# Arthur151/ROMP

Measured on NVIDIA H100. Metric: frames/sec 512x512 ROMP-HRNet32 (whole hot path), higher is better.
Workload: dtype bf16

## Files before the change

### romp_b200/csrc/conv_block_tc.cu

```cuda
#include "conv_tc.cuh"
#include "tc_device.cuh"

namespace b200romp {

namespace {

constexpr int kBlkThreads = 384;
constexpr int kRowB = 128;
constexpr int kHaloH = 20;
constexpr int kTapBytes = 64 * kRowB;
constexpr int kHalfTapBytes = 64 * 64;

template <bool FOLD>
struct BlkCfg {
  static constexpr int kWBytes = FOLD ? 3 * (kTapBytes + 2 * kHalfTapBytes) : 9 * kTapBytes;
  static constexpr int kTW = FOLD ? 16 : 8;
  static constexpr int kHaloW = kTW + 4;
  static constexpr int kN1 = FOLD ? 192 : 128;
  static constexpr int kN2 = 8 * kTW;
  static constexpr int kG2 = kN2 / 8;
  static constexpr int kMidRows = 2 * kN1;
  static constexpr int kStagePayload = kHaloH * kHaloW * kRowB;
  static constexpr int kStageBytes = ((kMidRows + 2 * kHaloW + 2) * kRowB + 1023) / 1024 * 1024;
  static constexpr int kMidBytes = kMidRows * kRowB;
  static constexpr int kSmemBytes = 2 * kWBytes + kStageBytes + kMidBytes + 1024  + 1024 ;
  static_assert(17 * kHaloW + kTW + 1 < kMidRows, "conv1 blocks do not cover the mid pixels conv2 reads");
  static_assert(kHaloH * kHaloW - 2 * kHaloW - 2 > 17 * kHaloW + kTW + 1, "an unwritten stage row feeds a mid row conv2 reads");
  static_assert(kSmemBytes <= 227 * 1024, "fused block does not fit shared memory");
  static_assert(kWBytes % kTapBytes == 0, "weights are copied in tap-sized pieces");
};

__host__ __device__ constexpr int w_tap_off(bool fold, int tap) {
  return !fold ? tap * kTapBytes
               : (tap / 3) * (kTapBytes + 2 * kHalfTapBytes) + (tap % 3 == 0 ? 0 : tap % 3 == 1 ? kHalfTapBytes : kHalfTapBytes + kTapBytes);
}

template <bool FOLD>
__device__ __forceinline__ constexpr bool blk_skip(int tap, int k) {
  return FOLD && ((tap % 3 == 0 && k < 2) || (tap % 3 == 2 && k >= 2));
}

template <bool FOLD>
__device__ __forceinline__ uint64_t w_desc(uint32_t w_base, int tap, int k) {
  const uint32_t t = w_base + (uint32_t)w_tap_off(FOLD, tap);
  if (FOLD && tap % 3 != 1) return make_smem_desc(t + (k & 1) * 32, 8 * 64, kSw64);
  return make_smem_desc(t + k * 32, 8 * kRowB, kSw128);
}

__device__ __forceinline__ void consumers_bar_sync() { asm volatile("bar.sync 1, 256;" ::: "memory"); }

__device__ __forceinline__ void ldmatrix_x4_trans(uint32_t (&r)[4], uint32_t addr) {
  asm volatile("ldmatrix.sync.aligned.m8n8.x4.trans.shared.b16 {%0, %1, %2, %3}, [%4];"
               : "=r"(r[0]), "=r"(r[1]), "=r"(r[2]), "=r"(r[3])
               : "r"(addr));
}
__device__ __forceinline__ void stmatrix_x4_trans(uint32_t addr, const uint32_t (&r)[4]) {
  asm volatile("stmatrix.sync.aligned.m8n8.x4.trans.shared.b16 [%0], {%1, %2, %3, %4};" ::"r"(addr), "r"(r[0]), "r"(r[1]), "r"(r[2]),
               "r"(r[3])
               : "memory");
}
__device__ __forceinline__ void st_shared_zero16(uint32_t addr) {
  asm volatile("st.shared.v4.b32 [%0], {%1, %1, %1, %1};" ::"r"(addr), "r"(0) : "memory");
}
template <int N>
__device__ __forceinline__ void wgmma_bf16(float (&d)[N / 2], uint64_t a, uint64_t b, uint32_t scale_d) {
  if constexpr (N == 192) wgmma_n192_bf16(d, a, b, scale_d);
  else if constexpr (N == 128) wgmma_n128_bf16(d, a, b, scale_d);
  else wgmma_n64(d, a, b, scale_d, false);
}
template <typename T>
__device__ __forceinline__ T opaque(T v) {
  uint64_t u = (uint64_t)v;
  asm volatile("mov.b64 %0, %0;" : "+l"(u));
  return (T)u;
}
__device__ __forceinline__ uint32_t pack_bf16x2(float a, float b) {
  const __nv_bfloat162 v = __floats2bfloat162_rn(a, b);
  return *reinterpret_cast<const uint32_t*>(&v);
}

struct BlkThread {
  int g, w, l;
};
template <bool FOLD>
__device__ __forceinline__ int c2_oy0(int g) { return FOLD ? 0 : 8 * g; }
template <bool FOLD>
__device__ __forceinline__ int c2_ox0(int g) { return FOLD ? 8 * g : 0; }
struct BlkTile {
  int n, y0, x0;
  __device__ BlkTile(int tile, int tiles_x, int per_frame, int tw) {
    n = tile / per_frame;
    const int rem = tile % per_frame;
    y0 = (rem / tiles_x) * 16;
    x0 = (rem % tiles_x) * tw;
  }
};

template <bool FOLD>
__device__ __forceinline__ void conv1_issue(float (&acc)[BlkCfg<FOLD>::kN1 / 2], uint32_t a_base, uint32_t w1_base, int row0) {
  constexpr int kHaloW = BlkCfg<FOLD>::kHaloW, kN1 = BlkCfg<FOLD>::kN1;
#pragma unroll
  for (int j = 0; j < kN1 / 2; ++j) acc[j] = 0.f;
  uint32_t scale_d = 0;
  wgmma_fence();
#pragma unroll
  for (int tap = 0; tap < 9; ++tap) {
    const uint32_t b_tap = a_base + (uint32_t)((row0 + (tap / 3) * kHaloW + tap % 3) * kRowB);
#pragma unroll
    for (int k = 0; k < 4; ++k) {
      if (blk_skip<FOLD>(tap, k)) continue;
      wgmma_bf16<kN1>(acc, w_desc<FOLD>(w1_base, tap, k), make_smem_desc(b_tap + k * 32, 8 * kRowB, kSw128), scale_d);
      scale_d = 1;
    }
  }
  wgmma_commit();
}

template <bool FOLD>
__device__ __forceinline__ void load_residual(uint32_t (&rv)[BlkCfg<FOLD>::kG2][2], uint32_t a_base, const BlkThread& th) {
  constexpr int kHaloW = BlkCfg<FOLD>::kHaloW;
  const int q = th.l >> 3;
#pragma unroll
  for (int j0 = 0; j0 < BlkCfg<FOLD>::kG2; j0 += 2) {
    const int hr = (c2_oy0<FOLD>(th.g) + j0 + (q >> 1) + 2) * kHaloW + c2_ox0<FOLD>(th.g) + (th.l & 7) + 2;
    uint32_t r[4];
    ldmatrix_x4_trans(r, a_base + hr * kRowB + (((2 * th.w + (q & 1)) ^ (hr & 7)) << 4));
    rv[j0][0] = r[0]; rv[j0][1] = r[1]; rv[j0 + 1][0] = r[2]; rv[j0 + 1][1] = r[3];
  }
}

template <bool FOLD>
__device__ __forceinline__ void mid_epilogue(const float (&acc)[BlkCfg<FOLD>::kN1 / 2], uint32_t mid_base, const float* b1p, const ConvParams& p,
                                             const BlkTile& tl, const BlkThread& th, int row0) {
  constexpr int kHaloW = BlkCfg<FOLD>::kHaloW, kTW = BlkCfg<FOLD>::kTW, kN1 = BlkCfg<FOLD>::kN1;
  const float bias[2] = {__ldg(b1p + 16 * th.w + (th.l >> 2)), __ldg(b1p + 16 * th.w + (th.l >> 2) + 8)};
  const int q = th.l >> 3;
#pragma unroll
  for (int j0 = 0; j0 < kN1 / 8; j0 += 2) {
    uint32_t r[4];
#pragma unroll
    for (int i = 0; i < 4; ++i) {
      const int j = j0 + (i >> 1), e = i & 1;
      r[i] = pack_bf16x2(fmaxf(acc[4 * j + 2 * e] + bias[e], 0.f), fmaxf(acc[4 * j + 2 * e + 1] + bias[e], 0.f));
    }
    const int m = row0 + 8 * (j0 + (q >> 1)) + (th.l & 7);
    stmatrix_x4_trans(mid_base + m * kRowB + (((2 * th.w + (q & 1)) ^ (m & 7)) << 4), r);
  }
  if (tl.y0 > 0 && tl.x0 > 0 && tl.y0 + 16 < p.Hout && tl.x0 + kTW < p.Wout) return;
  __syncwarp();
  constexpr int kRingRow = kTW + 2, kRing = 2 * kRingRow + 2 * 18;
#pragma unroll 1
  for (int i = th.l; i < 2 * kRing; i += 32) {
    const int k = i >> 1;
    const int my = k < 2 * kRingRow ? (k < kRingRow ? 0 : 17) : (k - 2 * kRingRow) % 18;
    const int mx = k < 2 * kRingRow ? k % kRingRow : (k - 2 * kRingRow < 18 ? 0 : kTW + 1);
    const int m = my * kHaloW + mx;
    if (m >= row0 && m < row0 + kN1 && ((unsigned)(tl.y0 - 1 + my) >= (unsigned)p.Hout || (unsigned)(tl.x0 - 1 + mx) >= (unsigned)p.Wout))
      st_shared_zero16(mid_base + m * kRowB + (((2 * th.w + (i & 1)) ^ (m & 7)) << 4));
  }
}

template <bool FOLD>
__device__ __forceinline__ void conv2_issue(float (&acc2)[BlkCfg<FOLD>::kN2 / 2], uint32_t mid_base, uint32_t w2_base, int g) {
  constexpr int kHaloW = BlkCfg<FOLD>::kHaloW, kN2 = BlkCfg<FOLD>::kN2;
#pragma unroll
  for (int j = 0; j < kN2 / 2; ++j) acc2[j] = 0.f;
  uint32_t scale_d = 0;
  wgmma_fence();
#pragma unroll
  for (int tap = 0; tap < 9; ++tap) {
    const uint32_t b_tap = mid_base + (uint32_t)(((c2_oy0<FOLD>(g) + tap / 3) * kHaloW + c2_ox0<FOLD>(g) + tap % 3) * kRowB);
#pragma unroll
    for (int k = 0; k < 4; ++k) {
      if (blk_skip<FOLD>(tap, k)) continue;
      wgmma_bf16<kN2>(acc2, w_desc<FOLD>(w2_base, tap, k), make_smem_desc(b_tap + k * 32, kHaloW * kRowB, kSw128), scale_d);
      scale_d = 1;
    }
  }
  wgmma_commit();
}

template <bool FOLD>
__device__ __forceinline__ void out_epilogue(const float (&acc2)[BlkCfg<FOLD>::kN2 / 2], const uint32_t (&rv)[BlkCfg<FOLD>::kG2][2],
                                             const float* b2p, const ConvParams& p, const BlkTile& tl, const BlkThread& th) {
  __nv_bfloat16* out = reinterpret_cast<__nv_bfloat16*>(p.out);
  const int c = 16 * th.w + (th.l >> 2);
  const float bias[2] = {__ldg(b2p + c), __ldg(b2p + c + 8)};
  const int odd = (th.l >> 2) & 1;
  const int x = tl.x0 + c2_ox0<FOLD>(th.g) + 2 * (th.l & 3) + odd;
#pragma unroll
  for (int j = 0; j < BlkCfg<FOLD>::kG2; ++j) {
    uint16_t h[2][2];
#pragma unroll
    for (int e = 0; e < 2; ++e) {
      const float2 r = res_pair(rv[j][e]);
      const float a = (acc2[4 * j + 2 * e] + bias[e]) + r.x, b = (acc2[4 * j + 2 * e + 1] + bias[e]) + r.y;
      h[e][0] = __bfloat16_as_ushort(__float2bfloat16_rn(fmaxf(a, 0.f)));
      h[e][1] = __bfloat16_as_ushort(__float2bfloat16_rn(fmaxf(b, 0.f)));
    }
    const uint32_t send = odd ? (uint32_t)h[0][0] | ((uint32_t)h[1][0] << 16) : (uint32_t)h[0][1] | ((uint32_t)h[1][1] << 16);
    const uint32_t recv = __shfl_xor_sync(0xffffffffu, send, 4);
    const size_t pix = ((size_t)tl.n * p.Hout + tl.y0 + c2_oy0<FOLD>(th.g) + j) * p.Wout + x;
    uint32_t* o = reinterpret_cast<uint32_t*>(out + pix * p.out_C + p.out_c_off + (c & ~1));
#pragma unroll
    for (int e = 0; e < 2; ++e) {
      const uint32_t theirs = (recv >> (16 * e)) & 0xFFFFu;
      o[4 * e] = odd ? (theirs | ((uint32_t)h[e][1] << 16)) : ((uint32_t)h[e][0] | (theirs << 16));
    }
  }
}

}

template <bool FOLD>
__global__ void __launch_bounds__(kBlkThreads, 1)
conv_block_tc_kernel(const __grid_constant__ CUtensorMap tmap, const ConvParams p, const uint8_t* __restrict__ w1pack,
                     const uint8_t* __restrict__ w2pack, const float* __restrict__ bias1, int tiles_x, int tiles_y, int num_tiles) {
  using Cfg = BlkCfg<FOLD>;
  constexpr int kWBytes = Cfg::kWBytes, kStageBytes = Cfg::kStageBytes;
  extern __shared__ uint8_t smem_raw[];
  uint8_t* smem = reinterpret_cast<uint8_t*>((reinterpret_cast<uintptr_t>(smem_raw) + 1023) & ~(uintptr_t)1023);
  uint8_t* sW1 = smem;
  uint8_t* sW2 = smem + kWBytes;
  uint8_t* sA = smem + 2 * kWBytes;
  uint8_t* sMid = sA + kStageBytes;
  uint64_t* full = reinterpret_cast<uint64_t*>(sMid + Cfg::kMidBytes);
  uint64_t* empty = full + 1;
  uint64_t* w_full = full + 2;

  const int warp = threadIdx.x >> 5;
  if (threadIdx.x == 0) {
    mbar_init(full, 1);
    mbar_init(empty, 256);
    mbar_init(w_full, 1);
    fence_barrier_init();
  }
  __syncthreads();
  pdl_trigger();
  const int per_frame = tiles_x * tiles_y;

  if (warp == 0) {
    if (elect_one()) {
      mbar_arrive_expect_tx(w_full, 2 * kWBytes);
      for (int off = 0; off < kWBytes; off += kTapBytes) {
        bulk_copy_g2s(sW1 + off, w1pack + off, kTapBytes, w_full);
        bulk_copy_g2s(sW2 + off, w2pack + off, kTapBytes, w_full);
      }
      pdl_wait();
      const uint64_t pol = l2_policy_stream();
      uint32_t phase = 0;
      for (int tile = blockIdx.x; tile < num_tiles; tile += gridDim.x, phase ^= 1) {
        const BlkTile tl(tile, tiles_x, per_frame, Cfg::kTW);
        mbar_wait(empty, phase ^ 1);
        mbar_arrive_expect_tx(full, Cfg::kStagePayload);
        tma_load_4d(sA, &tmap, full, 0, tl.x0 - 2, tl.y0 - 2, tl.n, pol);
      }
    }
  } else if (warp >= 4) {
    const int t = threadIdx.x & 127;
    const BlkThread th{(warp >> 2) - 1, t >> 5, t & 31};
    pdl_wait();
    mbar_wait(w_full, 0);
    float acc[Cfg::kN1 / 2], acc2[Cfg::kN2 / 2];
    uint32_t rv[Cfg::kG2][2];
    const int row0 = th.g * Cfg::kN1;
    uint32_t phase = 0;
    for (int tile = blockIdx.x; tile < num_tiles; tile += gridDim.x, phase ^= 1) {
      const uint32_t w1_base = opaque(smem_u32(sW1)), w2_base = opaque(smem_u32(sW2)), a_base = opaque(smem_u32(sA)),
                     mid_base = opaque(smem_u32(sMid));
      const float* b1p = opaque(bias1);
      const float* b2p = opaque(p.bias);
      const BlkTile tl(tile, tiles_x, per_frame, Cfg::kTW);
      mbar_wait(full, phase);
      conv1_issue<FOLD>(acc, a_base, w1_base, row0);
      load_residual<FOLD>(rv, a_base, th);
      wgmma_wait<0>();
      mbar_arrive(empty);
      consumers_bar_sync();
      mid_epilogue<FOLD>(acc, mid_base, b1p, p, tl, th, row0);
      fence_proxy_async();
      consumers_bar_sync();
      conv2_issue<FOLD>(acc2, mid_base, w2_base, th.g);
      wgmma_wait<0>();
      out_epilogue<FOLD>(acc2, rv, b2p, p, tl, th);
    }
  }
}

bool tc_block_supported(const ConvParams& p, bool fold) {
  if (p.in_dtype != B200ROMP_BF16 || p.out_dtype != B200ROMP_BF16 || p.res_dtype != B200ROMP_BF16) return false;
  if (p.cin != 64 || p.cout != 64 || p.up != 1 || p.out_nchw || p.pow_channel >= 0 || p.input_norm || !p.relu) return false;
  if (p.Hin != p.Hout || p.Win != p.Wout || p.Hout % 16 != 0 || p.Wout % (fold ? BlkCfg<true>::kTW : BlkCfg<false>::kTW) != 0) return false;
  if (p.in_C % 8 != 0 || p.in_c_off % 8 != 0 || p.out_C % 8 != 0 || p.out_c_off % 8 != 0) return false;
  if (p.res != p.in || p.res_C != p.in_C || p.res_c_off != p.in_c_off || p.res_broadcast) return false;
  return (reinterpret_cast<uintptr_t>(p.in) & 15) == 0;
}

static int block_pack_weights(const float* w_oihw, bool fold, void** d_out, std::vector<void*>* allocs) {
  if (!fold) return tc_pack_weights(w_oihw, 64, 64, 9, 64, d_out, allocs, kRowB, 2);
  const std::vector<uint8_t> full = tc_pack_image(w_oihw, 64, 64, 9, 64, kRowB, 2);
  const std::vector<uint8_t> half = tc_pack_image(w_oihw, 64, 64, 9, 64, 64, 2);
  std::vector<uint8_t> img(BlkCfg<true>::kWBytes);
  for (int tap = 0; tap < 9; ++tap) {
    uint8_t* dst = img.data() + w_tap_off(true, tap);
    if (tap % 3 == 1) memcpy(dst, full.data() + (size_t)tap * kTapBytes, kTapBytes);
    else memcpy(dst, half.data() + (size_t)(2 * tap + (tap % 3 == 0 ? 1 : 0)) * kHalfTapBytes, kHalfTapBytes);
  }
  *d_out = upload(img.data(), img.size(), allocs);
  return *d_out ? B200ROMP_OK : B200ROMP_ECUDA;
}

int tc_block_prepare(const ConvParams& p, const float* w1_oihw, const float* b1, const float* w2_oihw, int sm_count,
                     TcConvPlan* plan, std::vector<void*>* allocs) {
  plan->kind = 60;
  plan->eb = 2;
  plan->cin = plan->cout = plan->nt = 64;
  plan->grid_x = sm_count;
  plan->grid_y = 1;
  plan->stages = 1;
  plan->smem_bytes = plan->fold ? BlkCfg<true>::kSmemBytes : BlkCfg<false>::kSmemBytes;
  int rc = block_pack_weights(w1_oihw, plan->fold, &plan->d_wpack, allocs);
  if (rc) return rc;
  rc = block_pack_weights(w2_oihw, plan->fold, &plan->d_wpack2, allocs);
  if (rc) return rc;
  plan->d_bias1 = static_cast<const float*>(upload(b1, 64 * sizeof(float), allocs));
  if (!plan->d_bias1) return B200ROMP_ECUDA;
  rc = tc_encode_nhwc_input(&plan->tmap_in, p, 2, 64, plan->fold ? BlkCfg<true>::kHaloW : BlkCfg<false>::kHaloW, kHaloH,
                            CU_TENSOR_MAP_SWIZZLE_128B, "conv_block_tc");
  if (rc) return rc;
  B2R_CUDA_OK(cudaFuncSetAttribute(conv_block_tc_kernel<false>, cudaFuncAttributeMaxDynamicSharedMemorySize, BlkCfg<false>::kSmemBytes));
  B2R_CUDA_OK(cudaFuncSetAttribute(conv_block_tc_kernel<true>, cudaFuncAttributeMaxDynamicSharedMemorySize, BlkCfg<true>::kSmemBytes));
  return B200ROMP_OK;
}

int tc_block_launch(const TcConvPlan& plan, const ConvParams& p, cudaStream_t stream) {
  const int tiles_x = p.Wout / (plan.fold ? BlkCfg<true>::kTW : BlkCfg<false>::kTW), tiles_y = p.Hout / 16;
  const int num_tiles = tiles_x * tiles_y * p.B;
  const dim3 grid(std::min(plan.grid_x, num_tiles));
  auto kern = plan.fold ? conv_block_tc_kernel<true> : conv_block_tc_kernel<false>;
  B2R_CUDA_OK(tc_launch(kern, grid, kBlkThreads, plan.smem_bytes, stream, plan.tmap_in, p, reinterpret_cast<const uint8_t*>(plan.d_wpack),
                        reinterpret_cast<const uint8_t*>(plan.d_wpack2), plan.d_bias1, tiles_x, tiles_y, num_tiles));
  return B200ROMP_OK;
}

}
```

### romp_b200/csrc/conv_tc.cuh

```cuda
#pragma once
#include <cuda.h>

#include <string>
#include <vector>

#include "common.cuh"

namespace b200romp {

struct S2Maps {
  CUtensorMap m[4];
};

struct TcConvPlan {
  int kind = 0;
  int cin = 0, cout = 0, nt = 0;
  int eb = 2;
  int grid_x = 0, grid_y = 0, stages = 0;
  int smem_bytes = 0;
  void* d_wpack = nullptr;
  CUtensorMap tmap_in;
  S2Maps tmap_s2;
  unsigned kmask = 0xFFFFFFFFu;
  const void* encoded_in = nullptr;
  int encoded_batch = 0;
  void* d_wpack2 = nullptr;
  void* d_wpack3 = nullptr;
  const float* d_bias1 = nullptr;
  const float* d_bias2 = nullptr;
  int fold = 0;
  std::string describe() const;
};

bool tc_conv_supported(const ConvParams& p, int ksize, int stride);
int tc_conv_prepare(const ConvParams& p, int ksize, int stride, const float* w_oihw, int sm_count, TcConvPlan* plan,
                    std::vector<void*>* allocs);
int tc_conv_launch(const TcConvPlan& plan, const ConvParams& p, cudaStream_t stream);
bool tc_conv1d_supported(const ConvParams& p);
int tc_conv1d_prepare(const ConvParams& p, const float* w_oi3, int sm_count, TcConvPlan* plan, std::vector<void*>* allocs);
int tc_conv1d_launch(TcConvPlan& plan, const ConvParams& p, cudaStream_t stream);
bool tc_stem_supported(const ConvParams& p, int ksize, int stride);
int tc_stem_prepare(const ConvParams& p, const float* w_oihw, int sm_count, TcConvPlan* plan, std::vector<void*>* allocs);
int tc_stem_launch(const TcConvPlan& plan, const ConvParams& p, cudaStream_t stream);
bool tc_block_supported(const ConvParams& p, bool fold);
int tc_block_prepare(const ConvParams& p, const float* w1_oihw, const float* b1, const float* w2_oihw, int sm_count,
                     TcConvPlan* plan, std::vector<void*>* allocs);
int tc_block_launch(const TcConvPlan& plan, const ConvParams& p, cudaStream_t stream);
struct BottleneckMids {
  __nv_bfloat16* t1 = nullptr;
  __nv_bfloat16* t2 = nullptr;
  int t1_C = 0, t2_C = 0;
};
bool tc_bottleneck_supported(const ConvParams& p);
int tc_bottleneck_prepare(const ConvParams& p, const float* w1_oihw, const float* b1, const float* w2_oihw, const float* b2,
                          const float* w3_oihw, int sm_count, TcConvPlan* plan, std::vector<void*>* allocs);
int tc_bottleneck_launch(const TcConvPlan& plan, const ConvParams& p, const BottleneckMids& mids, cudaStream_t stream);

}
```

### romp_b200/csrc/net.cu

```cuda
#include <stdarg.h>
#include <stdlib.h>
#include <string.h>

#include <algorithm>
#include <array>
#include <map>
#include <mutex>
#include <vector>

#include "common.cuh"
#include "conv_tc.cuh"

namespace b200romp {

static thread_local std::string g_last_error;

void set_error(const char* fmt, ...) {
  char buf[1024];
  va_list ap;
  va_start(ap, fmt);
  vsnprintf(buf, sizeof(buf), fmt, ap);
  va_end(ap);
  g_last_error = buf;
}
// ... 786 lines not shown
    snprintf(line, sizeof(line), "op%03zu %s k%d s%d %4d->%-4d in t%d[%dx%dx%d]+%d out t%d[%dx%dx%d]+%d res t%d up%d relu%d%s\n", i,
             on_wgmma(kernel) ? "wgmma  " : "simt   ", d.ksize, d.stride, d.cin, d.cout, d.in, ti.H, ti.W, ti.C, d.in_c_off, d.out,
             to.H, to.W, to.C, d.out_c_off, d.res, d.upsample, d.relu, bracket);
    s += line;
  };
  for (size_t i = 0; i < net->ops.size(); ++i) {
    const Op& op = net->ops[i];
    const b200romp_conv_desc& d = op.d;
    const Tensor& ti = net->tensors[d.in];
    const Tensor& to = net->tensors[d.out];
    switch (op.kernel) {
      case Kernel::MaxPool:
        snprintf(line, sizeof(line), "op%03zu maxpool 3x3 s2 in t%d[%dx%dx%d] out t%d[%dx%dx%d]\n", i, d.in, ti.H, ti.W, ti.C, d.out, to.H, to.W, to.C);
        s += line;
        break;
      case Kernel::Sum: {
        int n = snprintf(line, sizeof(line), "op%03zu sum     out t%d[%dx%dx%d] = relu%d( t%d", i, op.sum.out, to.H, to.W, to.C, op.sum.relu, op.sum.base);
        for (int k = 0; k < op.sum.n_terms; ++k) n += snprintf(line + n, sizeof(line) - n, " + up%d(t%d)", op.sum.up[k], op.sum.term[k]);
        n += snprintf(line + n, sizeof(line) - n, " )");
        bool bound = net->finalized && to.ptr && ti.ptr;
        for (int k = 0; k < op.sum.n_terms; ++k) bound = bound && net->tensors[op.sum.term[k]].ptr;
        SumParams sp;
        if (bound && fill_sum_params(net, op, net->max_batch, &sp) == B200ROMP_OK)
          n += snprintf(line + n, sizeof(line) - n, " [fuse-sum %s]", fuse_sum_kernel_name(sp));
        snprintf(line + n, sizeof(line) - n, "\n");
        s += line;
        break;
      }
      case Kernel::WgmmaBlock: {
        const int mid = op.parts[0].d.out;
        const Tensor& tm = net->tensors[mid];
        snprintf(line, sizeof(line),
                 "op%03zu wgmma   block k3 s1 %d->%d->%d in t%d[%dx%dx%d]+%d mid t%d[%dx%dx%d] out t%d[%dx%dx%d]+%d res t%d+%d up1 relu1 "
                 "bias1 bias2 [tc-block grid %d smem %d%s]\n",
                 i, d.cin, d.cin, d.cout, d.in, ti.H, ti.W, ti.C, d.in_c_off, mid, tm.H, tm.W, tm.C, d.out, to.H, to.W, to.C,
                 d.out_c_off, d.res, d.res_c_off, op.tc.grid_x, op.tc.smem_bytes, op.tc.fold ? " conv1 pixel-pairs conv2 pixel-pairs" : "");
        s += line;
        break;
      }
      case Kernel::WgmmaBottleneck:
        for (size_t k = 0; k < op.parts.size(); ++k) {
          char bracket[96];
          snprintf(bracket, sizeof(bracket), " [tc-bottleneck conv%zu of k1-k3-k1 grid %d smem %d]", k + 1, op.tc.grid_x, op.tc.smem_bytes);
          conv_line(i, op.parts[k].d, op.kernel, bracket);
        }
        break;
      default:
        conv_line(i, d, op.kernel, on_wgmma(op.kernel) ? op.tc.describe().c_str() : "");
    }
  }
  snprintf(line, sizeof(line), "workspace %.1f MiB for max_batch %d\n", net->workspace_bytes / 1048576.0, net->max_batch);
  s += line;
  const int n = (int)std::min<size_t>(s.size(), (size_t)len - 1);
  memcpy(buf, s.data(), n);
  buf[n] = 0;
  return n;
}

int b200romp_net_set_lane(b200romp_net* net, int op, int lane) {
  B2R_REQUIRE(net && !net->finalized && op >= 0 && op < (int)net->ops.size(), "set_lane: bad op id or net already finalized");
  B2R_REQUIRE(lane >= 0 && lane < b200romp_net::kLanes, "set_lane: lane must be 0..%d", b200romp_net::kLanes - 1);
  net->ops[op].lane = lane;
  return B200ROMP_OK;
}

int b200romp_net_num_launches(b200romp_net* net) { return net ? (int)net->ops.size() : 0; }
long long b200romp_net_workspace_bytes(b200romp_net* net) { return net ? (long long)net->workspace_bytes : 0; }

int b200romp_conv2d(const b200romp_conv_desc* d, const float* weight_host, const float* bias_host, const void* in,
// ... 47 lines not shown
```

### romp_b200/csrc/tc_device.cuh

```cuda
#pragma once
#include <cuda.h>

#include <vector>

#include "conv_tc.cuh"

namespace b200romp {

__device__ __forceinline__ uint32_t smem_u32(const void* p) { return (uint32_t)__cvta_generic_to_shared(p); }

__device__ __forceinline__ void mbar_init(uint64_t* bar, uint32_t count) {
  asm volatile("mbarrier.init.shared::cta.b64 [%0], %1;" ::"r"(smem_u32(bar)), "r"(count) : "memory");
}
__device__ __forceinline__ void mbar_arrive_expect_tx(uint64_t* bar, uint32_t bytes) {
  asm volatile("mbarrier.arrive.expect_tx.shared::cta.b64 _, [%0], %1;" ::"r"(smem_u32(bar)), "r"(bytes) : "memory");
}
__device__ __forceinline__ void mbar_arrive(uint64_t* bar) {
  asm volatile("mbarrier.arrive.shared::cta.b64 _, [%0];" ::"r"(smem_u32(bar)) : "memory");
}
__device__ __forceinline__ bool mbar_try_wait(uint64_t* bar, uint32_t parity) {
  uint32_t ok;
  asm volatile(
      "{\n\t.reg .pred p;\n\t"
      "mbarrier.try_wait.parity.shared::cta.b64 p, [%1], %2;\n\t"
// ... 26 lines not shown
  asm volatile("createpolicy.fractional.L2::evict_normal.b64 %0, 1.0;" : "=l"(pol));
  return pol;
}
__device__ __forceinline__ void tma_load_3d(void* dst, const CUtensorMap* map, uint64_t* bar, int c0, int c1, int c2, uint64_t pol) {
  asm volatile(
      "cp.async.bulk.tensor.3d.shared::cluster.global.mbarrier::complete_tx::bytes.L2::cache_hint [%0], [%1, {%3, %4, %5}], [%2], %6;"
      ::"r"(smem_u32(dst)), "l"(map), "r"(smem_u32(bar)), "r"(c0), "r"(c1), "r"(c2), "l"(pol)
      : "memory");
}
__device__ __forceinline__ void tma_load_4d(void* dst, const CUtensorMap* map, uint64_t* bar, int c0, int c1, int c2, int c3, uint64_t pol) {
  asm volatile(
      "cp.async.bulk.tensor.4d.shared::cluster.global.mbarrier::complete_tx::bytes.L2::cache_hint [%0], [%1, {%3, %4, %5, %6}], [%2], %7;"
      ::"r"(smem_u32(dst)), "l"(map), "r"(smem_u32(bar)), "r"(c0), "r"(c1), "r"(c2), "r"(c3), "l"(pol)
      : "memory");
}
__device__ __forceinline__ void tma_load_5d(void* dst, const CUtensorMap* map, uint64_t* bar, int c0, int c1, int c2, int c3,
                                            int c4, uint64_t pol) {
  asm volatile(
      "cp.async.bulk.tensor.5d.shared::cluster.global.mbarrier::complete_tx::bytes.L2::cache_hint [%0], [%1, {%3, %4, %5, %6, %7}], [%2], %8;"
      ::"r"(smem_u32(dst)), "l"(map), "r"(smem_u32(bar)), "r"(c0), "r"(c1), "r"(c2), "r"(c3), "r"(c4), "l"(pol)
      : "memory");
}
__device__ __forceinline__ void bulk_copy_g2s(void* dst, const void* src, uint32_t bytes, uint64_t* bar) {
  asm volatile("cp.async.bulk.shared::cluster.global.mbarrier::complete_tx::bytes [%0], [%1], %2, [%3];"
               ::"r"(smem_u32(dst)), "l"(src), "r"(bytes), "r"(smem_u32(bar))
               : "memory");
}

__device__ __forceinline__ void wgmma_fence() { asm volatile("wgmma.fence.sync.aligned;" ::: "memory"); }
__device__ __forceinline__ void wgmma_commit() { asm volatile("wgmma.commit_group.sync.aligned;" ::: "memory"); }
template <int N>
__device__ __forceinline__ void wgmma_wait() { asm volatile("wgmma.wait_group.sync.aligned %0;" ::"n"(N) : "memory"); }

#define B2R_WG_R8(i) "+f"(d[i + 0]), "+f"(d[i + 1]), "+f"(d[i + 2]), "+f"(d[i + 3]), "+f"(d[i + 4]), "+f"(d[i + 5]), "+f"(d[i + 6]), "+f"(d[i + 7])
__device__ __forceinline__ void wgmma_n16(float (&d)[8], uint64_t a, uint64_t b, uint32_t scale_d, bool tf32) {
  if (!tf32)
    asm volatile(
        "{\n\t.reg .pred p;\n\tsetp.ne.b32 p, %10, 0;\n\t"
        "wgmma.mma_async.sync.aligned.m64n16k16.f32.bf16.bf16 {%0, %1, %2, %3, %4, %5, %6, %7}, %8, %9, p, 1, 1, 0, 0;\n\t}"
        : B2R_WG_R8(0)
        : "l"(a), "l"(b), "r"(scale_d)
        : "memory");
  else
    asm volatile(
        "{\n\t.reg .pred p;\n\tsetp.ne.b32 p, %10, 0;\n\t"
        "wgmma.mma_async.sync.aligned.m64n16k8.f32.tf32.tf32 {%0, %1, %2, %3, %4, %5, %6, %7}, %8, %9, p, 1, 1;\n\t}"
        : B2R_WG_R8(0)
        : "l"(a), "l"(b), "r"(scale_d)
        : "memory");
}
__device__ __forceinline__ void wgmma_n32(float (&d)[16], uint64_t a, uint64_t b, uint32_t scale_d, bool tf32) {
  if (!tf32)
    asm volatile(
        "{\n\t.reg .pred p;\n\tsetp.ne.b32 p, %18, 0;\n\t"
        "wgmma.mma_async.sync.aligned.m64n32k16.f32.bf16.bf16 {%0, %1, %2, %3, %4, %5, %6, %7, %8, %9, %10, %11, %12, %13, %14, %15}, "
        "%16, %17, p, 1, 1, 0, 0;\n\t}"
        : B2R_WG_R8(0), B2R_WG_R8(8)
        : "l"(a), "l"(b), "r"(scale_d)
        : "memory");
  else
    asm volatile(
        "{\n\t.reg .pred p;\n\tsetp.ne.b32 p, %18, 0;\n\t"
        "wgmma.mma_async.sync.aligned.m64n32k8.f32.tf32.tf32 {%0, %1, %2, %3, %4, %5, %6, %7, %8, %9, %10, %11, %12, %13, %14, %15}, "
        "%16, %17, p, 1, 1;\n\t}"
        : B2R_WG_R8(0), B2R_WG_R8(8)
        : "l"(a), "l"(b), "r"(scale_d)
        : "memory");
}
__device__ __forceinline__ void wgmma_n64(float (&d)[32], uint64_t a, uint64_t b, uint32_t scale_d, bool tf32) {
  if (!tf32)
    asm volatile(
        "{\n\t.reg .pred p;\n\tsetp.ne.b32 p, %34, 0;\n\t"
        "wgmma.mma_async.sync.aligned.m64n64k16.f32.bf16.bf16 {%0, %1, %2, %3, %4, %5, %6, %7, %8, %9, %10, %11, %12, %13, %14, "
        "%15, %16, %17, %18, %19, %20, %21, %22, %23, %24, %25, %26, %27, %28, %29, %30, %31}, %32, %33, p, 1, 1, 0, 0;\n\t}"
        : B2R_WG_R8(0), B2R_WG_R8(8), B2R_WG_R8(16), B2R_WG_R8(24)
        : "l"(a), "l"(b), "r"(scale_d)
        : "memory");
  else
    asm volatile(
        "{\n\t.reg .pred p;\n\tsetp.ne.b32 p, %34, 0;\n\t"
        "wgmma.mma_async.sync.aligned.m64n64k8.f32.tf32.tf32 {%0, %1, %2, %3, %4, %5, %6, %7, %8, %9, %10, %11, %12, %13, %14, "
        "%15, %16, %17, %18, %19, %20, %21, %22, %23, %24, %25, %26, %27, %28, %29, %30, %31}, %32, %33, p, 1, 1;\n\t}"
        : B2R_WG_R8(0), B2R_WG_R8(8), B2R_WG_R8(16), B2R_WG_R8(24)
        : "l"(a), "l"(b), "r"(scale_d)
        : "memory");
}
__device__ __forceinline__ void wgmma_n128_bf16(float (&d)[64], uint64_t a, uint64_t b, uint32_t scale_d) {
  asm volatile(
      "{\n\t.reg .pred p;\n\tsetp.ne.b32 p, %66, 0;\n\t"
      "wgmma.mma_async.sync.aligned.m64n128k16.f32.bf16.bf16 {%0, %1, %2, %3, %4, %5, %6, %7, %8, %9, %10, %11, %12, %13, %14, "
      "%15, %16, %17, %18, %19, %20, %21, %22, %23, %24, %25, %26, %27, %28, %29, %30, %31, %32, %33, %34, %35, %36, %37, %38, "
      "%39, %40, %41, %42, %43, %44, %45, %46, %47, %48, %49, %50, %51, %52, %53, %54, %55, %56, %57, %58, %59, %60, %61, %62, "
      "%63}, %64, %65, p, 1, 1, 0, 0;\n\t}"
      : B2R_WG_R8(0), B2R_WG_R8(8), B2R_WG_R8(16), B2R_WG_R8(24), B2R_WG_R8(32), B2R_WG_R8(40), B2R_WG_R8(48), B2R_WG_R8(56)
      : "l"(a), "l"(b), "r"(scale_d)
      : "memory");
}
__device__ __forceinline__ void wgmma_n192_bf16(float (&d)[96], uint64_t a, uint64_t b, uint32_t scale_d) {
  asm volatile(
      "{\n\t.reg .pred p;\n\tsetp.ne.b32 p, %98, 0;\n\t"
      "wgmma.mma_async.sync.aligned.m64n192k16.f32.bf16.bf16 {%0, %1, %2, %3, %4, %5, %6, %7, %8, %9, %10, %11, %12, %13, %14, "
      "%15, %16, %17, %18, %19, %20, %21, %22, %23, %24, %25, %26, %27, %28, %29, %30, %31, %32, %33, %34, %35, %36, %37, %38, "
      "%39, %40, %41, %42, %43, %44, %45, %46, %47, %48, %49, %50, %51, %52, %53, %54, %55, %56, %57, %58, %59, %60, %61, %62, "
      "%63, %64, %65, %66, %67, %68, %69, %70, %71, %72, %73, %74, %75, %76, %77, %78, %79, %80, %81, %82, %83, %84, %85, %86, "
      "%87, %88, %89, %90, %91, %92, %93, %94, %95}, %96, %97, p, 1, 1, 0, 0;\n\t}"
      : B2R_WG_R8(0), B2R_WG_R8(8), B2R_WG_R8(16), B2R_WG_R8(24), B2R_WG_R8(32), B2R_WG_R8(40), B2R_WG_R8(48), B2R_WG_R8(56),
        B2R_WG_R8(64), B2R_WG_R8(72), B2R_WG_R8(80), B2R_WG_R8(88)
      : "l"(a), "l"(b), "r"(scale_d)
      : "memory");
}
#undef B2R_WG_R8
template <int NT, int EB>
__device__ __forceinline__ void wgmma_any(float (&d)[NT / 2], uint64_t a, uint64_t b, uint32_t scale_d) {
  if constexpr (NT == 64) wgmma_n64(d, a, b, scale_d, EB == 4);
  else if constexpr (NT == 32) wgmma_n32(d, a, b, scale_d, EB == 4);
  else wgmma_n16(d, a, b, scale_d, EB == 4);
}

constexpr uint32_t kSw128 = 1, kSw64 = 2;
__device__ __forceinline__ uint64_t make_smem_desc(uint32_t addr, uint32_t sbo_bytes, uint32_t layout) {
  return (uint64_t)((addr & 0x3FFFF) >> 4) | ((uint64_t)1 << 16) | ((uint64_t)(sbo_bytes >> 4) << 32) | ((uint64_t)layout << 62);
}
__host__ __device__ constexpr uint32_t tc_layout(int row_bytes) { return row_bytes == 128 ? kSw128 : kSw64; }

__host__ __device__ constexpr int tc_row_bytes(int ksize, int cin, int eb) {
  return (ksize == 3 && cin >= 128) ? 64 : (cin * eb < 128 ? cin * eb : 128);
}

__device__ __forceinline__ uint32_t tf32_rna(uint32_t x) {
  uint32_t y;
  asm("cvt.rna.tf32.f32 %0, %1;" : "=r"(y) : "r"(x));
  return y;
}
__device__ __forceinline__ void tf32_round_smem(uint8_t* base, int bytes, int t, int nthreads) {
  const uint32_t s0 = smem_u32(base);
  for (int off = t * 16; off < bytes; off += nthreads * 16) {
    uint32_t a, b, c, d;
    asm volatile("ld.shared.v4.b32 {%0, %1, %2, %3}, [%4];" : "=r"(a), "=r"(b), "=r"(c), "=r"(d) : "r"(s0 + off));
    a = tf32_rna(a); b = tf32_rna(b); c = tf32_rna(c); d = tf32_rna(d);
    asm volatile("st.shared.v4.b32 [%4], {%0, %1, %2, %3};" ::"r"(a), "r"(b), "r"(c), "r"(d), "r"(s0 + off) : "memory");
  }
}

__device__ __forceinline__ void wg_store2(const ConvParams& p, int n, int oy, int ox, int co, float v0, float v1) {
// ... 198 lines not shown
```

Baseline: 3714.

## Reuse conv1 halo rows across vertically adjacent tiles in fused block strips

Each CTA now walks a vertical strip of tiles. For every tile after the first, it carries the bottom two halo rows of the mid (conv1) output into the top of the buffer and recomputes conv1 only for the new rows, using smaller wgmma N sizes (96/112/56/32 instead of 128/192). This cuts redundant conv1 halo recomputation. The cost is more complex control flow, extra smem loads and stores for the carried rows, and coarser work units that can leave SMs load-imbalanced (the strip picker tries to avoid this).

```diff
diff --git a/romp_b200/csrc/conv_block_tc.cu b/romp_b200/csrc/conv_block_tc.cu
--- a/romp_b200/csrc/conv_block_tc.cu
+++ b/romp_b200/csrc/conv_block_tc.cu
@@ -16,15 +16,25 @@
   static constexpr int kWBytes = FOLD ? 3 * (kTapBytes + 2 * kHalfTapBytes) : 9 * kTapBytes;
   static constexpr int kTW = FOLD ? 16 : 8;
   static constexpr int kHaloW = kTW + 4;
-  static constexpr int kN1 = FOLD ? 192 : 128;
+  static constexpr int kCarry = 2 * kHaloW;
+  static constexpr int kN1F = FOLD ? 128 : 112, kN1FB = FOLD ? 56 : 0;
+  static constexpr int kN1C = FOLD ? 128 : 96, kN1CB = FOLD ? 32 : 0;
   static constexpr int kN2 = 8 * kTW;
   static constexpr int kG2 = kN2 / 8;
-  static constexpr int kMidRows = 2 * kN1;
+  static constexpr int kMidRows = 2 * (kN1F + kN1FB);
+  static constexpr int kAcc1 = (kN1F + kN1FB) / 2;
+  static constexpr int kCarryChunks = kCarry * kRowB / 16;
   static constexpr int kStagePayload = kHaloH * kHaloW * kRowB;
   static constexpr int kStageBytes = ((kMidRows + 2 * kHaloW + 2) * kRowB + 1023) / 1024 * 1024;
   static constexpr int kMidBytes = kMidRows * kRowB;
   static constexpr int kSmemBytes = 2 * kWBytes + kStageBytes + kMidBytes + 1024  + 1024 ;
-  static_assert(17 * kHaloW + kTW + 1 < kMidRows, "conv1 blocks do not cover the mid pixels conv2 reads");
+  static_assert(17 * kHaloW + kTW + 1 < kMidRows, "conv1 of a strip's first tile does not cover the mid pixels conv2 reads");
+  static_assert(17 * kHaloW + kTW + 1 < kCarry + 2 * (kN1C + kN1CB), "conv1 of a continuing tile does not cover the mid pixels conv2 reads");
+  static_assert(kCarry + 2 * (kN1C + kN1CB) <= kMidRows, "conv1 of a continuing tile writes past the mid buffer");
+  static_assert(kN1C + kN1CB <= kN1F + kN1FB, "conv1 accumulators sized for the first tile");
+  static_assert(kCarry % 8 == 0 && (16 * kHaloW) % 8 == 0 && kN1F % 8 == 0 && kN1C % 8 == 0 && kN1FB % 8 == 0 && kN1CB % 8 == 0,
+                "conv1 ranges and the carried rows must start on 8-row swizzle phases");
+  static_assert(kStagePayload <= kStageBytes, "the halo does not fit the stage");
   static_assert(kHaloH * kHaloW - 2 * kHaloW - 2 > 17 * kHaloW + kTW + 1, "an unwritten stage row feeds a mid row conv2 reads");
   static_assert(kSmemBytes <= 227 * 1024, "fused block does not fit shared memory");
   static_assert(kWBytes % kTapBytes == 0, "weights are copied in tap-sized pieces");
@@ -59,14 +69,36 @@
                "r"(r[3])
                : "memory");
 }
+__device__ __forceinline__ void stmatrix_x2_trans(uint32_t addr, uint32_t r0, uint32_t r1) {
+  asm volatile("stmatrix.sync.aligned.m8n8.x2.trans.shared.b16 [%0], {%1, %2};" ::"r"(addr), "r"(r0), "r"(r1) : "memory");
+}
 __device__ __forceinline__ void st_shared_zero16(uint32_t addr) {
   asm volatile("st.shared.v4.b32 [%0], {%1, %1, %1, %1};" ::"r"(addr), "r"(0) : "memory");
 }
+__device__ __forceinline__ uint4 ld_shared16(uint32_t addr) {
+  uint4 v;
+  asm volatile("ld.shared.v4.b32 {%0, %1, %2, %3}, [%4];" : "=r"(v.x), "=r"(v.y), "=r"(v.z), "=r"(v.w) : "r"(addr) : "memory");
+  return v;
+}
+__device__ __forceinline__ void st_shared16(uint32_t addr, uint4 v) {
+  asm volatile("st.shared.v4.b32 [%0], {%1, %2, %3, %4};" ::"r"(addr), "r"(v.x), "r"(v.y), "r"(v.z), "r"(v.w) : "memory");
+}
 template <int N>
 __device__ __forceinline__ void wgmma_bf16(float (&d)[N / 2], uint64_t a, uint64_t b, uint32_t scale_d) {
-  if constexpr (N == 192) wgmma_n192_bf16(d, a, b, scale_d);
-  else if constexpr (N == 128) wgmma_n128_bf16(d, a, b, scale_d);
-  else wgmma_n64(d, a, b, scale_d, false);
+  if constexpr (N == 128) wgmma_n128_bf16(d, a, b, scale_d);
+  else if constexpr (N == 112) wgmma_n112_bf16(d, a, b, scale_d);
+  else if constexpr (N == 96) wgmma_n96_bf16(d, a, b, scale_d);
+  else if constexpr (N == 64) wgmma_n64(d, a, b, scale_d, false);
+  else if constexpr (N == 56) wgmma_n56_bf16(d, a, b, scale_d);
+  else {
+    static_assert(N == 32, "no wgmma wrapper for this N");
+    wgmma_n32(d, a, b, scale_d, false);
+  }
+}
+template <int N, int OFF, int M>
+__device__ __forceinline__ float (&acc_slice(float (&acc)[M]))[N / 2] {
+  static_assert(OFF + N / 2 <= M, "accumulator array too small");
+  return *reinterpret_cast<float(*)[N / 2]>(&acc[OFF]);
 }
 template <typename T>
 __device__ __forceinline__ T opaque(T v) {
@@ -88,29 +120,43 @@
 __device__ __forceinline__ int c2_ox0(int g) { return FOLD ? 8 * g : 0; }
 struct BlkTile {
   int n, y0, x0;
-  __device__ BlkTile(int tile, int tiles_x, int per_frame, int tw) {
-    n = tile / per_frame;
-    const int rem = tile % per_frame;
-    y0 = (rem / tiles_x) * 16;
+  __device__ BlkTile(int seg, int k, int tiles_x, int segs_y, int strip, int tw) {
+    n = seg / (tiles_x * segs_y);
+    const int rem = seg % (tiles_x * segs_y);
+    y0 = ((rem / tiles_x) * strip + k) * 16;
     x0 = (rem % tiles_x) * tw;
   }
 };
 
-template <bool FOLD>
-__device__ __forceinline__ void conv1_issue(float (&acc)[BlkCfg<FOLD>::kN1 / 2], uint32_t a_base, uint32_t w1_base, int row0) {
-  constexpr int kHaloW = BlkCfg<FOLD>::kHaloW, kN1 = BlkCfg<FOLD>::kN1;
-#pragma unroll
-  for (int j = 0; j < kN1 / 2; ++j) acc[j] = 0.f;
+template <bool FOLD, int N, int NB, int M>
+__device__ __forceinline__ void conv1_issue(float (&acc)[M], uint32_t a_base, uint32_t w1_base, int row0, int row0b) {
+  constexpr int kHaloW = BlkCfg<FOLD>::kHaloW;
+#pragma unroll
+  for (int j = 0; j < (N + NB) / 2; ++j) acc[j] = 0.f;
+  wgmma_fence();
   uint32_t scale_d = 0;
-  wgmma_fence();
 #pragma unroll
   for (int tap = 0; tap < 9; ++tap) {
     const uint32_t b_tap = a_base + (uint32_t)((row0 + (tap / 3) * kHaloW + tap % 3) * kRowB);
 #pragma unroll
     for (int k = 0; k < 4; ++k) {
       if (blk_skip<FOLD>(tap, k)) continue;
-      wgmma_bf16<kN1>(acc, w_desc<FOLD>(w1_base, tap, k), make_smem_desc(b_tap + k * 32, 8 * kRowB, kSw128), scale_d);
+      wgmma_bf16<N>(acc_slice<N, 0>(acc), w_desc<FOLD>(w1_base, tap, k), make_smem_desc(b_tap + k * 32, 8 * kRowB, kSw128), scale_d);
       scale_d = 1;
+    }
+  }
+  if constexpr (NB > 0) {
+    scale_d = 0;
+#pragma unroll
+    for (int tap = 0; tap < 9; ++tap) {
+      const uint32_t b_tap = a_base + (uint32_t)((row0b + (tap / 3) * kHaloW + tap % 3) * kRowB);
+#pragma unroll
+      for (int k = 0; k < 4; ++k) {
+        if (blk_skip<FOLD>(tap, k)) continue;
+        wgmma_bf16<NB>(acc_slice<NB, N / 2>(acc), w_desc<FOLD>(w1_base, tap, k), make_smem_desc(b_tap + k * 32, 8 * kRowB, kSw128),
+                       scale_d);
+        scale_d = 1;
+      }
     }
   }
   wgmma_commit();
@@ -129,22 +175,24 @@
   }
 }
 
-template <bool FOLD>
-__device__ __forceinline__ void mid_epilogue(const float (&acc)[BlkCfg<FOLD>::kN1 / 2], uint32_t mid_base, const float* b1p, const ConvParams& p,
+template <bool FOLD, int N>
+__device__ __forceinline__ void mid_epilogue(const float (&acc)[N / 2], uint32_t mid_base, const float* b1p, const ConvParams& p,
                                              const BlkTile& tl, const BlkThread& th, int row0) {
-  constexpr int kHaloW = BlkCfg<FOLD>::kHaloW, kTW = BlkCfg<FOLD>::kTW, kN1 = BlkCfg<FOLD>::kN1;
+  constexpr int kHaloW = BlkCfg<FOLD>::kHaloW, kTW = BlkCfg<FOLD>::kTW;
   const float bias[2] = {__ldg(b1p + 16 * th.w + (th.l >> 2)), __ldg(b1p + 16 * th.w + (th.l >> 2) + 8)};
   const int q = th.l >> 3;
 #pragma unroll
-  for (int j0 = 0; j0 < kN1 / 8; j0 += 2) {
+  for (int j0 = 0; j0 < N / 8; j0 += 2) {
     uint32_t r[4];
 #pragma unroll
     for (int i = 0; i < 4; ++i) {
       const int j = j0 + (i >> 1), e = i & 1;
-      r[i] = pack_bf16x2(fmaxf(acc[4 * j + 2 * e] + bias[e], 0.f), fmaxf(acc[4 * j + 2 * e + 1] + bias[e], 0.f));
+      r[i] = j < N / 8 ? pack_bf16x2(fmaxf(acc[4 * j + 2 * e] + bias[e], 0.f), fmaxf(acc[4 * j + 2 * e + 1] + bias[e], 0.f)) : 0u;
     }
     const int m = row0 + 8 * (j0 + (q >> 1)) + (th.l & 7);
-    stmatrix_x4_trans(mid_base + m * kRowB + (((2 * th.w + (q & 1)) ^ (m & 7)) << 4), r);
+    const uint32_t addr = mid_base + m * kRowB + (((2 * th.w + (q & 1)) ^ (m & 7)) << 4);
+    if (j0 + 1 < N / 8) stmatrix_x4_trans(addr, r);
+    else stmatrix_x2_trans(addr, r[0], r[1]);
   }
   if (tl.y0 > 0 && tl.x0 > 0 && tl.y0 + 16 < p.Hout && tl.x0 + kTW < p.Wout) return;
   __syncwarp();
@@ -155,7 +203,7 @@
     const int my = k < 2 * kRingRow ? (k < kRingRow ? 0 : 17) : (k - 2 * kRingRow) % 18;
     const int mx = k < 2 * kRingRow ? k % kRingRow : (k - 2 * kRingRow < 18 ? 0 : kTW + 1);
     const int m = my * kHaloW + mx;
-    if (m >= row0 && m < row0 + kN1 && ((unsigned)(tl.y0 - 1 + my) >= (unsigned)p.Hout || (unsigned)(tl.x0 - 1 + mx) >= (unsigned)p.Wout))
+    if (m >= row0 && m < row0 + N && ((unsigned)(tl.y0 - 1 + my) >= (unsigned)p.Hout || (unsigned)(tl.x0 - 1 + mx) >= (unsigned)p.Wout))
       st_shared_zero16(mid_base + m * kRowB + (((2 * th.w + (i & 1)) ^ (m & 7)) << 4));
   }
 }
@@ -215,7 +263,7 @@
 template <bool FOLD>
 __global__ void __launch_bounds__(kBlkThreads, 1)
 conv_block_tc_kernel(const __grid_constant__ CUtensorMap tmap, const ConvParams p, const uint8_t* __restrict__ w1pack,
-                     const uint8_t* __restrict__ w2pack, const float* __restrict__ bias1, int tiles_x, int tiles_y, int num_tiles) {
+                     const uint8_t* __restrict__ w2pack, const float* __restrict__ bias1, int tiles_x, int segs_y, int strip, int num_segs) {
   using Cfg = BlkCfg<FOLD>;
   constexpr int kWBytes = Cfg::kWBytes, kStageBytes = Cfg::kStageBytes;
   extern __shared__ uint8_t smem_raw[];
@@ -237,7 +285,6 @@
   }
   __syncthreads();
   pdl_trigger();
-  const int per_frame = tiles_x * tiles_y;
 
   if (warp == 0) {
     if (elect_one()) {
@@ -249,11 +296,13 @@
       pdl_wait();
       const uint64_t pol = l2_policy_stream();
       uint32_t phase = 0;
-      for (int tile = blockIdx.x; tile < num_tiles; tile += gridDim.x, phase ^= 1) {
-        const BlkTile tl(tile, tiles_x, per_frame, Cfg::kTW);
-        mbar_wait(empty, phase ^ 1);
-        mbar_arrive_expect_tx(full, Cfg::kStagePayload);
-        tma_load_4d(sA, &tmap, full, 0, tl.x0 - 2, tl.y0 - 2, tl.n, pol);
+      for (int seg = blockIdx.x; seg < num_segs; seg += gridDim.x) {
+        for (int k = 0; k < strip; ++k, phase ^= 1) {
+          const BlkTile tl(seg, k, tiles_x, segs_y, strip, Cfg::kTW);
+          mbar_wait(empty, phase ^ 1);
+          mbar_arrive_expect_tx(full, Cfg::kStagePayload);
+          tma_load_4d(sA, &tmap, full, 0, tl.x0 - 2, tl.y0 - 2, tl.n, pol);
+        }
       }
     }
   } else if (warp >= 4) {
@@ -261,28 +310,49 @@
     const BlkThread th{(warp >> 2) - 1, t >> 5, t & 31};
     pdl_wait();
     mbar_wait(w_full, 0);
-    float acc[Cfg::kN1 / 2], acc2[Cfg::kN2 / 2];
+    constexpr int kN1F = Cfg::kN1F, kN1FB = Cfg::kN1FB, kN1C = Cfg::kN1C, kN1CB = Cfg::kN1CB;
+    float acc[Cfg::kAcc1], acc2[Cfg::kN2 / 2];
     uint32_t rv[Cfg::kG2][2];
-    const int row0 = th.g * Cfg::kN1;
+    constexpr int kCarryRegs = (Cfg::kCarryChunks + 255) / 256;
+    uint4 carry[kCarryRegs];
+    const int ct = 128 * th.g + t;
     uint32_t phase = 0;
-    for (int tile = blockIdx.x; tile < num_tiles; tile += gridDim.x, phase ^= 1) {
-      const uint32_t w1_base = opaque(smem_u32(sW1)), w2_base = opaque(smem_u32(sW2)), a_base = opaque(smem_u32(sA)),
-                     mid_base = opaque(smem_u32(sMid));
-      const float* b1p = opaque(bias1);
-      const float* b2p = opaque(p.bias);
-      const BlkTile tl(tile, tiles_x, per_frame, Cfg::kTW);
-      mbar_wait(full, phase);
-      conv1_issue<FOLD>(acc, a_base, w1_base, row0);
-      load_residual<FOLD>(rv, a_base, th);
-      wgmma_wait<0>();
-      mbar_arrive(empty);
-      consumers_bar_sync();
-      mid_epilogue<FOLD>(acc, mid_base, b1p, p, tl, th, row0);
-      fence_proxy_async();
-      consumers_bar_sync();
-      conv2_issue<FOLD>(acc2, mid_base, w2_base, th.g);
-      wgmma_wait<0>();
-      out_epilogue<FOLD>(acc2, rv, b2p, p, tl, th);
+    for (int seg = blockIdx.x; seg < num_segs; seg += gridDim.x) {
+      for (int k = 0; k < strip; ++k, phase ^= 1) {
+        const uint32_t w1_base = opaque(smem_u32(sW1)), w2_base = opaque(smem_u32(sW2)), a_base = opaque(smem_u32(sA)),
+                       mid_base = opaque(smem_u32(sMid));
+        const float* b1p = opaque(bias1);
+        const float* b2p = opaque(p.bias);
+        const BlkTile tl(seg, k, tiles_x, segs_y, strip, Cfg::kTW);
+        mbar_wait(full, phase);
+        if (k == 0) conv1_issue<FOLD, kN1F, kN1FB>(acc, a_base, w1_base, th.g * kN1F, 2 * kN1F + th.g * kN1FB);
+        else conv1_issue<FOLD, kN1C, kN1CB>(acc, a_base, w1_base, Cfg::kCarry + th.g * kN1C, Cfg::kCarry + 2 * kN1C + th.g * kN1CB);
+        load_residual<FOLD>(rv, a_base, th);
+        if (k > 0) {
+#pragma unroll
+          for (int i = 0; i < kCarryRegs; ++i)
+            if (ct + 256 * i < Cfg::kCarryChunks) carry[i] = ld_shared16(mid_base + 16 * kRowB * Cfg::kHaloW + 16 * (ct + 256 * i));
+        }
+        wgmma_wait<0>();
+        mbar_arrive(empty);
+        consumers_bar_sync();
+        if (k == 0) {
+          mid_epilogue<FOLD, kN1F>(acc_slice<kN1F, 0>(acc), mid_base, b1p, p, tl, th, th.g * kN1F);
+          if constexpr (kN1FB > 0) mid_epilogue<FOLD, kN1FB>(acc_slice<kN1FB, kN1F / 2>(acc), mid_base, b1p, p, tl, th, 2 * kN1F + th.g * kN1FB);
+        } else {
+#pragma unroll
+          for (int i = 0; i < kCarryRegs; ++i)
+            if (ct + 256 * i < Cfg::kCarryChunks) st_shared16(mid_base + 16 * (ct + 256 * i), carry[i]);
+          mid_epilogue<FOLD, kN1C>(acc_slice<kN1C, 0>(acc), mid_base, b1p, p, tl, th, Cfg::kCarry + th.g * kN1C);
+          if constexpr (kN1CB > 0) mid_epilogue<FOLD, kN1CB>(acc_slice<kN1CB, kN1C / 2>(acc), mid_base, b1p, p, tl, th,
+                                                              Cfg::kCarry + 2 * kN1C + th.g * kN1CB);
+        }
+        fence_proxy_async();
+        consumers_bar_sync();
+        conv2_issue<FOLD>(acc2, mid_base, w2_base, th.g);
+        wgmma_wait<0>();
+        out_epilogue<FOLD>(acc2, rv, b2p, p, tl, th);
+      }
     }
   }
 }
@@ -310,6 +380,18 @@
   return *d_out ? B200ROMP_OK : B200ROMP_ECUDA;
 }
 
+static int block_strip(int tiles_y, int num_tiles, int grid) {
+  const int most = (num_tiles + grid - 1) / grid;
+  for (int strip = tiles_y; strip > 1; --strip)
+    if (tiles_y % strip == 0 && (num_tiles / strip + grid - 1) / grid * strip <= most) return strip;
+  return 1;
+}
+
+static void block_tiles(const ConvParams& p, bool fold, int* tiles_x, int* tiles_y) {
+  *tiles_x = p.Wout / (fold ? BlkCfg<true>::kTW : BlkCfg<false>::kTW);
+  *tiles_y = p.Hout / 16;
+}
+
 int tc_block_prepare(const ConvParams& p, const float* w1_oihw, const float* b1, const float* w2_oihw, int sm_count,
                      TcConvPlan* plan, std::vector<void*>* allocs) {
   plan->kind = 60;
@@ -319,6 +401,9 @@
   plan->grid_y = 1;
   plan->stages = 1;
   plan->smem_bytes = plan->fold ? BlkCfg<true>::kSmemBytes : BlkCfg<false>::kSmemBytes;
+  int tiles_x, tiles_y;
+  block_tiles(p, plan->fold, &tiles_x, &tiles_y);
+  plan->strip = block_strip(tiles_y, tiles_x * tiles_y * p.B, sm_count);
   int rc = block_pack_weights(w1_oihw, plan->fold, &plan->d_wpack, allocs);
   if (rc) return rc;
   rc = block_pack_weights(w2_oihw, plan->fold, &plan->d_wpack2, allocs);
@@ -334,12 +419,15 @@
 }
 
 int tc_block_launch(const TcConvPlan& plan, const ConvParams& p, cudaStream_t stream) {
-  const int tiles_x = p.Wout / (plan.fold ? BlkCfg<true>::kTW : BlkCfg<false>::kTW), tiles_y = p.Hout / 16;
+  int tiles_x, tiles_y;
+  block_tiles(p, plan.fold, &tiles_x, &tiles_y);
   const int num_tiles = tiles_x * tiles_y * p.B;
-  const dim3 grid(std::min(plan.grid_x, num_tiles));
+  const int strip = block_strip(tiles_y, num_tiles, plan.grid_x);
+  const int segs_y = tiles_y / strip, num_segs = num_tiles / strip;
+  const dim3 grid(std::min(plan.grid_x, num_segs));
   auto kern = plan.fold ? conv_block_tc_kernel<true> : conv_block_tc_kernel<false>;
   B2R_CUDA_OK(tc_launch(kern, grid, kBlkThreads, plan.smem_bytes, stream, plan.tmap_in, p, reinterpret_cast<const uint8_t*>(plan.d_wpack),
-                        reinterpret_cast<const uint8_t*>(plan.d_wpack2), plan.d_bias1, tiles_x, tiles_y, num_tiles));
+                        reinterpret_cast<const uint8_t*>(plan.d_wpack2), plan.d_bias1, tiles_x, segs_y, strip, num_segs));
   return B200ROMP_OK;
 }
 
diff --git a/romp_b200/csrc/conv_tc.cuh b/romp_b200/csrc/conv_tc.cuh
--- a/romp_b200/csrc/conv_tc.cuh
+++ b/romp_b200/csrc/conv_tc.cuh
@@ -29,6 +29,7 @@
   const float* d_bias1 = nullptr;
   const float* d_bias2 = nullptr;
   int fold = 0;
+  int strip = 1;
   std::string describe() const;
 };
 
diff --git a/romp_b200/csrc/net.cu b/romp_b200/csrc/net.cu
--- a/romp_b200/csrc/net.cu
+++ b/romp_b200/csrc/net.cu
@@ -842,9 +842,10 @@
         const Tensor& tm = net->tensors[mid];
         snprintf(line, sizeof(line),
                  "op%03zu wgmma   block k3 s1 %d->%d->%d in t%d[%dx%dx%d]+%d mid t%d[%dx%dx%d] out t%d[%dx%dx%d]+%d res t%d+%d up1 relu1 "
-                 "bias1 bias2 [tc-block grid %d smem %d%s]\n",
+                 "bias1 bias2 [tc-block grid %d smem %d%s] strip %d\n",
                  i, d.cin, d.cin, d.cout, d.in, ti.H, ti.W, ti.C, d.in_c_off, mid, tm.H, tm.W, tm.C, d.out, to.H, to.W, to.C,
-                 d.out_c_off, d.res, d.res_c_off, op.tc.grid_x, op.tc.smem_bytes, op.tc.fold ? " conv1 pixel-pairs conv2 pixel-pairs" : "");
+                 d.out_c_off, d.res, d.res_c_off, op.tc.grid_x, op.tc.smem_bytes, op.tc.fold ? " conv1 pixel-pairs conv2 pixel-pairs" : "",
+                 op.tc.strip);
         s += line;
         break;
       }
diff --git a/romp_b200/csrc/tc_device.cuh b/romp_b200/csrc/tc_device.cuh
--- a/romp_b200/csrc/tc_device.cuh
+++ b/romp_b200/csrc/tc_device.cuh
@@ -82,6 +82,7 @@
 template <int N>
 __device__ __forceinline__ void wgmma_wait() { asm volatile("wgmma.wait_group.sync.aligned %0;" ::"n"(N) : "memory"); }
 
+#define B2R_WG_R4(i) "+f"(d[i + 0]), "+f"(d[i + 1]), "+f"(d[i + 2]), "+f"(d[i + 3])
 #define B2R_WG_R8(i) "+f"(d[i + 0]), "+f"(d[i + 1]), "+f"(d[i + 2]), "+f"(d[i + 3]), "+f"(d[i + 4]), "+f"(d[i + 5]), "+f"(d[i + 6]), "+f"(d[i + 7])
 __device__ __forceinline__ void wgmma_n16(float (&d)[8], uint64_t a, uint64_t b, uint32_t scale_d, bool tf32) {
   if (!tf32)
@@ -146,20 +147,38 @@
       : "l"(a), "l"(b), "r"(scale_d)
       : "memory");
 }
-__device__ __forceinline__ void wgmma_n192_bf16(float (&d)[96], uint64_t a, uint64_t b, uint32_t scale_d) {
-  asm volatile(
-      "{\n\t.reg .pred p;\n\tsetp.ne.b32 p, %98, 0;\n\t"
-      "wgmma.mma_async.sync.aligned.m64n192k16.f32.bf16.bf16 {%0, %1, %2, %3, %4, %5, %6, %7, %8, %9, %10, %11, %12, %13, %14, "
-      "%15, %16, %17, %18, %19, %20, %21, %22, %23, %24, %25, %26, %27, %28, %29, %30, %31, %32, %33, %34, %35, %36, %37, %38, "
-      "%39, %40, %41, %42, %43, %44, %45, %46, %47, %48, %49, %50, %51, %52, %53, %54, %55, %56, %57, %58, %59, %60, %61, %62, "
-      "%63, %64, %65, %66, %67, %68, %69, %70, %71, %72, %73, %74, %75, %76, %77, %78, %79, %80, %81, %82, %83, %84, %85, %86, "
-      "%87, %88, %89, %90, %91, %92, %93, %94, %95}, %96, %97, p, 1, 1, 0, 0;\n\t}"
-      : B2R_WG_R8(0), B2R_WG_R8(8), B2R_WG_R8(16), B2R_WG_R8(24), B2R_WG_R8(32), B2R_WG_R8(40), B2R_WG_R8(48), B2R_WG_R8(56),
-        B2R_WG_R8(64), B2R_WG_R8(72), B2R_WG_R8(80), B2R_WG_R8(88)
+__device__ __forceinline__ void wgmma_n96_bf16(float (&d)[48], uint64_t a, uint64_t b, uint32_t scale_d) {
+  asm volatile(
+      "{\n\t.reg .pred p;\n\tsetp.ne.b32 p, %50, 0;\n\t"
+      "wgmma.mma_async.sync.aligned.m64n96k16.f32.bf16.bf16 {%0, %1, %2, %3, %4, %5, %6, %7, %8, %9, %10, %11, %12, %13, "
+      "%14, %15, %16, %17, %18, %19, %20, %21, %22, %23, %24, %25, %26, %27, %28, %29, %30, %31, %32, %33, %34, %35, %36, "
+      "%37, %38, %39, %40, %41, %42, %43, %44, %45, %46, %47}, %48, %49, p, 1, 1, 0, 0;\n\t}"
+      : B2R_WG_R8(0), B2R_WG_R8(8), B2R_WG_R8(16), B2R_WG_R8(24), B2R_WG_R8(32), B2R_WG_R8(40)
       : "l"(a), "l"(b), "r"(scale_d)
       : "memory");
 }
+__device__ __forceinline__ void wgmma_n112_bf16(float (&d)[56], uint64_t a, uint64_t b, uint32_t scale_d) {
+  asm volatile(
+      "{\n\t.reg .pred p;\n\tsetp.ne.b32 p, %58, 0;\n\t"
+      "wgmma.mma_async.sync.aligned.m64n112k16.f32.bf16.bf16 {%0, %1, %2, %3, %4, %5, %6, %7, %8, %9, %10, %11, %12, %13, "
+      "%14, %15, %16, %17, %18, %19, %20, %21, %22, %23, %24, %25, %26, %27, %28, %29, %30, %31, %32, %33, %34, %35, %36, "
+      "%37, %38, %39, %40, %41, %42, %43, %44, %45, %46, %47, %48, %49, %50, %51, %52, %53, %54, %55}, %56, %57, p, 1, 1, "
+      "0, 0;\n\t}"
+      : B2R_WG_R8(0), B2R_WG_R8(8), B2R_WG_R8(16), B2R_WG_R8(24), B2R_WG_R8(32), B2R_WG_R8(40), B2R_WG_R8(48)
+      : "l"(a), "l"(b), "r"(scale_d)
+      : "memory");
+}
+__device__ __forceinline__ void wgmma_n56_bf16(float (&d)[28], uint64_t a, uint64_t b, uint32_t scale_d) {
+  asm volatile(
+      "{\n\t.reg .pred p;\n\tsetp.ne.b32 p, %30, 0;\n\t"
+      "wgmma.mma_async.sync.aligned.m64n56k16.f32.bf16.bf16 {%0, %1, %2, %3, %4, %5, %6, %7, %8, %9, %10, %11, %12, %13, "
+      "%14, %15, %16, %17, %18, %19, %20, %21, %22, %23, %24, %25, %26, %27}, %28, %29, p, 1, 1, 0, 0;\n\t}"
+      : B2R_WG_R8(0), B2R_WG_R8(8), B2R_WG_R8(16), B2R_WG_R4(24)
+      : "l"(a), "l"(b), "r"(scale_d)
+      : "memory");
+}
 #undef B2R_WG_R8
+#undef B2R_WG_R4
 template <int NT, int EB>
 __device__ __forceinline__ void wgmma_any(float (&d)[NT / 2], uint64_t a, uint64_t b, uint32_t scale_d) {
   if constexpr (NT == 64) wgmma_n64(d, a, b, scale_d, EB == 4);
```

Result: no change. 3679, median of 6 (-0.9%).
